# lazytiger/pbrt-rs

Hardware: AMD Instinct MI355X
Metric: Mrays/s (higher is better)
Workload: dtype f32

## Files before the change

### pbrt-rs_amd/csrc/render.hip

```cpp
#include <hip/hip_runtime.h>
#include "abi_guard.h"

#include <algorithm>
#include <chrono>
#include <cstdio>
#include <cstdlib>
#include <cstring>
#include <string>
#include <thread>
#include <vector>

#include "scene.h"
#include "trace.h"
#include "wavefront.h"

using namespace pb;

extern "C" int pbrt_hip_render_device(PbrtHipScene* s, const PbrtCamera* camera, const PbrtRenderParams* params,
                                      float* d_film, PbrtRenderStats* stats) try {
    if (!s || !camera || !params || !d_film) return PBRT_HIP_ERR_INVALID;
    PB_ENTER(s->ctx);
    HIP_TRY(s->ctx, hipSetDevice(s->ctx->device));
    return wavefront_render(s, *camera, *params, d_film, stats);
}
// ... 509 lines not shown
        if (stats) *stats = local;
        return PBRT_HIP_OK;
    }
    const int n_pix = (int)origins.size() * kTile * kTile;
    int64_t valid_pixels = 0;
    for (const int2& o : origins)
        valid_pixels += (int64_t)(std::min(o.x + kTile, rp.x1) - o.x) * (std::min(o.y + kTile, rp.y1) - o.y);
    if (li_mode) valid_pixels = li->n;
    if (export_mode) rp.spp_per_pass = rp.spp;
    int spp_pass = rp.spp_per_pass > 0 ? rp.spp_per_pass : 0;
    if (spp_pass == 0) {
        size_t free_b = 0, total_b = 0;
        HIP_TRY(ctx, hipMemGetInfo(&free_b, &total_b));
        for (const auto& b : ctx->block_cache)
            if (!b.in_use) free_b += b.bytes;
        const int64_t per_path = 400 + (rp.integrator != PBRT_INTEGRATOR_PATH ? 24 + 48ll * std::max(1, rp.max_depth) : 0);
        const int64_t target_paths = std::max<int64_t>(1ll << 20, std::min<int64_t>(1ll << 28, (int64_t)(free_b / 2) / per_path));
        spp_pass = (int)std::max<int64_t>(1, std::min<int64_t>(rp.spp, target_paths / n_pix));
    }
    spp_pass = std::min(spp_pass, rp.spp);
    if (export_mode && spp_pass != rp.spp) return invalid("camera rays: too many samples for one pass");
    const size_t N = (size_t)n_pix * spp_pass;
    if (N * 4 >= (1ull << 32)) return invalid("too many concurrent paths for 32-bit queue entries; lower spp_per_pass");

    DevBuf buf(ctx);
    bool ok = true;
    PathState ps;
    ps.n_paths = N;
    ps.two_level = s->d.bvh.instanced ? 1 : 0;
    ps.ray = buf.alloc<float4>(N * 6, &ok);
    ps.hit = buf.alloc<float4>(N * 6, &ok);
    ps.rng = buf.alloc<uint64_t>(N, &ok);
    ps.L = buf.alloc<float4>(N, &ok);
    ps.beta = buf.alloc<float4>(N, &ok);
    ps.nee_a = buf.alloc<float4>(N, &ok);
    ps.nee_f = buf.alloc<float4>(N, &ok);
    ps.nee_b = buf.alloc<float4>(N, &ok);
    ps.nee_light = buf.alloc<int>(N, &ok);
    ps.pfilm = buf.alloc<float2>(N, &ok);
    Queues q[2];
    for (int k = 0; k < 2; ++k) {
        q[k].trace = buf.alloc<uint32_t>(N * 3, &ok);
        q[k].shade = buf.alloc<uint32_t>(N, &ok);
        q[k].counts64 = buf.alloc<unsigned long long>(2, &ok);
        q[k].keys = nullptr;
        for (int a = 0; a < 3; ++a) {
// ... 462 lines not shown
```

### pbrt-rs_amd/csrc/wf_direct.h

```cpp
#pragma once
#include "wf_path.h"

namespace pb {

struct DirectState {
    int* stage;
    float4* ld_acc;
    float4* frames;
    int light_strategy;
    int mode;
    int ao_samples;
    int ao_cos_sample;
};

#ifndef PB_DIRECT_WAVES
#define PB_DIRECT_WAVES 2
#endif
template <int MODE>
__global__ void __launch_bounds__(256, PB_DIRECT_WAVES) k_shade_direct(ShadeConsts sc, PathState ps, DirectState ds, Queues qin,
                                                        Queues qout, PassParams pp, TileList tiles, uint32_t n_in) {
    uint32_t i = blockIdx.x * blockDim.x + threadIdx.x;
    bool active = i < n_in;
    uint32_t p = active ? qin.shade[i] : 0u;
    bool emit_cont = false, emit_mis = false, emit_shadow = false, mis_bool = false;
    if (active && !(__float_as_int(ps.beta[p].w) & PF_VALID)) active = false;

    if (active) {
        float4 Lq = ps.L[p], bq = ps.beta[p];
        V3 L = V3{Lq.x, Lq.y, Lq.z};
        V3 T = V3{bq.x, bq.y, bq.z};
        int fb = __float_as_int(bq.w);
        int flags = fb & 0xff, depth = fb >> 8;
        int sg = ds.stage[p];
        int stage = sg & 0xffff, sp = sg >> 16;
        float4 accq = ds.ld_acc[p];
        V3 ld_acc = V3{accq.x, accq.y, accq.z};
        size_t rbase = ray_index(ps, p, RS_CONT), hbase = hit_index(ps, p, RS_CONT);
        constexpr int mode = MODE;
        const bool sample_all = mode == PBRT_INTEGRATOR_DIRECT && ds.light_strategy == 0;
        Samp sm = path_sampler(ps, pp, tiles, p);
        const bool tabulated = pp.smp.kind != PBRT_SAMPLER_RANDOM;
        bool fallback = (sm.arr & 0x8000) != 0;
        auto stages_at_vertex = [&]() {
            return (mode == PBRT_INTEGRATOR_AO)        ? ds.ao_samples
                   : (sc.n_lights == 0)                ? 0
                   : (mode == PBRT_INTEGRATOR_WHITTED) ? sc.n_lights
                   : !sample_all                       ? 1
// ... 216 lines not shown
            }
            if (branched) break;
            if (sp == 0) {
                done = true;
                break;
            }
            sp -= 1;
            size_t fi = ((size_t)p * pp.max_depth + sp) * 3;
            float4 f0 = ds.frames[fi], f1 = ds.frames[fi + 1], f2 = ds.frames[fi + 2];
            float4 r0 = ps.ray[rbase];
            ps.ray[rbase] = make_float4(r0.x, r0.y, r0.z, f0.x);
            ps.ray[rbase + 1] = make_float4(f0.y, f0.z, kInf, 0.0f);
            ps.hit[hbase] = make_float4(f1.z, f0.w, f1.x, f1.y);
            if (ps.two_level) ps.hit[hbase + 1] = make_float4(f2.w, 0.0f, 0.0f, 0.0f);
            depth = __float_as_int(f1.w);
            T = V3{f2.x, f2.y, f2.z};
            stage = total + 1;
            surface_ready = false;
            have_vertex = true;
        }
        samp_store(ps, p, sm);
        ps.L[p] = make_float4(L.x, L.y, L.z, 1.0f);
        ps.beta[p] = make_float4(T.x, T.y, T.z, __int_as_float((depth << 8) | flags));
        ds.stage[p] = (stage & 0xffff) | (sp << 16);
        ds.ld_acc[p] = make_float4(ld_acc.x, ld_acc.y, ld_acc.z, 0.0f);
    }

    __shared__ BlockAppend sh;
    block_append(sh, qout, p, emit_cont, emit_mis, emit_shadow, emit_cont || emit_mis || emit_shadow, 0, mis_bool);
}

}
```

### pbrt-rs_amd/csrc/wf_generate_trace.h

```cpp
#pragma once
#include "wf_sampler.h"

namespace pb {

__global__ void k_generate(PathState ps, Queues q, PassParams pp, DevCamera cam, TileList tiles) {
    uint32_t p = blockIdx.x * blockDim.x + threadIdx.x;
    uint32_t n = (uint32_t)pp.n_pix * pp.n_samples;
    if (p >= n) return;
    int s_local, pix;
    path_to_sample_pixel(pp, p, &s_local, &pix);
    int tile = pix >> 8, within = pix & 255;
    int2 org = tiles.origin[tile];
    int x = org.x + (within & 15), y = org.y + (within >> 4);
    bool valid = x >= pp.x0 && x < pp.x1 && y >= pp.y0 && y < pp.y1;
    int flags = 0;
    if (valid) {
        int s = pp.sample0 + s_local;
        Samp sm;
        rng_set_sequence(sm.rng, sample_sequence(pp, x, y, s));
        sm.pix = pix;
        sm.s = s;
        sm.dim1 = sm.dim2 = sm.arr = 0;
        sm.h_offset = pp.smp.kind == PBRT_SAMPLER_HALTON ? halton_pixel_offset(pp.smp, x, y) : 0;
        float u0, u1, l0, l1;
// ... 43 lines not shown
        float xa = __builtin_fabsf(m[0] * o.x) + __builtin_fabsf(m[1] * o.y) + __builtin_fabsf(m[2] * o.z) + __builtin_fabsf(m[3]);
        float ya = __builtin_fabsf(m[4] * o.x) + __builtin_fabsf(m[5] * o.y) + __builtin_fabsf(m[6] * o.z) + __builtin_fabsf(m[7]);
        float za = __builtin_fabsf(m[8] * o.x) + __builtin_fabsf(m[9] * o.y) + __builtin_fabsf(m[10] * o.z) + __builtin_fabsf(m[11]);
        V3 o_err = V3{xa, ya, za} * kGamma3;
        V3 dw = xform_vector(m, d);
        float l2 = len2(dw);
        float tmax = kInf;
        if (l2 > 0.0f) {
            float dt = dot(vabs(dw), o_err) / l2;
            ow = ow + dw * dt;
            tmax -= dt;
        }
        store_ray(ps, p, RS_CONT, ow, dw, tmax);
        samp_store(ps, p, sm);
        ps.pfilm[p] = make_float2(pfx, pfy);
        flags = PF_VALID | PF_ALIVE;
    } else {
        ps.pfilm[p] = make_float2(0.0f, 0.0f);
    }
    ps.L[p] = make_float4(0.0f, 0.0f, 0.0f, 1.0f);
    ps.beta[p] = make_float4(1.0f, 1.0f, 1.0f, __int_as_float(flags));
    if (!valid) store_ray(ps, p, RS_CONT, V3{0.0f, 0.0f, 0.0f}, V3{0.0f, 0.0f, 1.0f}, -1.0f);
    q.trace[p] = p * 4u + RS_CONT;
    q.shade[p] = p;
}

__global__ void k_li_generate(PathState ps, Queues q, const PbrtRay* __restrict__ rays, const uint64_t* __restrict__ keys, uint32_t n,
                              uint32_t n_padded, int skip) {
    uint32_t p = blockIdx.x * blockDim.x + threadIdx.x;
    if (p >= n_padded) return;
    int flags = 0;
    if (p < n) {
        Rng rng;
        rng_set_sequence(rng, keys[p]);
        for (int k = 0; k < skip; ++k) (void)rng_u32(rng);
        ps.rng[p] = rng.state;
        ps.samp[p] = 0;
        const float4* rp = reinterpret_cast<const float4*>(rays + p);
        float4 a = rp[0], b = rp[1];
        store_ray(ps, p, RS_CONT, V3{a.x, a.y, a.z}, V3{a.w, b.x, b.y}, b.z);
        flags = PF_VALID | PF_ALIVE;
    } else {
        store_ray(ps, p, RS_CONT, V3{0.0f, 0.0f, 0.0f}, V3{0.0f, 0.0f, 1.0f}, -1.0f);
    }
    ps.pfilm[p] = make_float2(0.0f, 0.0f);
    ps.L[p] = make_float4(0.0f, 0.0f, 0.0f, 1.0f);
    ps.beta[p] = make_float4(1.0f, 1.0f, 1.0f, __int_as_float(flags));
    q.trace[p] = p * 4u + RS_CONT;
    q.shade[p] = p;
}
__global__ void k_li_output(PathState ps, uint32_t n, float* __restrict__ rgb) {
    uint32_t p = blockIdx.x * blockDim.x + threadIdx.x;
    if (p >= n) return;
    float4 L = ps.L[p];
    rgb[3 * (size_t)p] = L.x;
    rgb[3 * (size_t)p + 1] = L.y;
    rgb[3 * (size_t)p + 2] = L.z;
}
__global__ void k_camera_rays_out(PathState ps, PassParams pp, TileList tiles, PbrtRay* __restrict__ rays, uint64_t* __restrict__ keys,
                                  float* __restrict__ pfilm, int32_t* __restrict__ pixel_sample) {
    uint32_t p = blockIdx.x * blockDim.x + threadIdx.x;
    uint32_t n = (uint32_t)pp.n_pix * pp.n_samples;
    if (p >= n) return;
    int s_local, pix;
    path_to_sample_pixel(pp, p, &s_local, &pix);
    int2 org = tiles.origin[pix >> 8];
    int x = org.x + (pix & 15), y = org.y + ((pix & 255) >> 4);
    bool valid = (__float_as_int(ps.beta[p].w) & PF_VALID) != 0;
    size_t ri = ray_index(ps, p, RS_CONT);
    float4 a = ps.ray[ri], b = ps.ray[ri + 1];
    float4* out = reinterpret_cast<float4*>(rays + p);
    out[0] = a;
// ... 84 lines not shown
```

### pbrt-rs_amd/csrc/wf_lights.h

```cpp
#pragma once
#include "wf_surface.h"

namespace pb {

PB_DEV V3 sphere_through(V3 v) {
    return V3{1.0f * v.x + 0.0f * v.y + 0.0f * v.z, 0.0f * v.x + 1.0f * v.y + 0.0f * v.z, 0.0f * v.x + 0.0f * v.y + 1.0f * v.z};
}
PB_DEV float sphere_area(float radius) { return (360.0f * (kPi / 180.0f)) * radius * (radius - (-radius)); }
PB_DEV void sphere_light_sample(float cx, float cy, float cz, float radius, const Surf& sf, float u0, float u1, V3* p_o,
                                V3* err_o, V3* n_o, float* pdf_o) {
    V3 pc = V3{1.0f * 0.0f + 0.0f * 0.0f + 0.0f * 0.0f + cx, 0.0f * 0.0f + 1.0f * 0.0f + 0.0f * 0.0f + cy,
               0.0f * 0.0f + 0.0f * 0.0f + 1.0f * 0.0f + cz};
    V3 p_origin = offset_ray_origin(sf.p, sf.p_error, sf.n, pc - sf.p);
    if (len2(p_origin - pc) <= radius * radius) {
        float z = 1.0f - 2.0f * u0;
        float rr = __builtin_sqrtf(fmaxr(1.0f - z * z, 0.0f));
        float sp, cp;
        det_sincos(2.0f * kPi * u1, &sp, &cp);
        V3 obj = V3{rr * cp, rr * sp, z} * radius;
        V3 n = normalize(sphere_through(obj));
        obj = obj * (radius / length(obj));
        V3 oe = vabs(obj) * kGamma5;
        const float g3 = kGamma3;
        V3 p = V3{1.0f * obj.x + 0.0f * obj.y + 0.0f * obj.z + cx, 0.0f * obj.x + 1.0f * obj.y + 0.0f * obj.z + cy,
// ... 296 lines not shown
                iu = iu < 0 ? 0 : (iu > 1 ? 1 : iu);
                int iv = (int)(theta * kInvPi * 2.0f);
                iv = iv < 0 ? 0 : (iv > 1 ? 1 : iv);
                lpdf = sc.env_cond_func[iv][iu] / sc.env_marg_int / (2.0f * kPi * kPi * st);
            }
        }
        if (lpdf != 0.0f) {
            float weight = power_heuristic1(spdf, lpdf);
            V3 o2 = offset_ray_origin(sf.p, sf.p_error, sf.n, wi2);
            store_ray(ps, p, RS_MIS, o2, wi2, kInf);
            ps.nee_f[p] = make_float4(f2.x, f2.y, f2.z, weight);
            nee_flags |= PF_NEE_MIS;
            if (sc.mis_bool && lt.type != PBRT_LIGHT_DIFFUSE_AREA) nee_flags |= NEE_MIS_BOOL;
        }
    }
    if (nee_flags) {
        ps.nee_a[p] = make_float4(A.x, A.y, A.z, pick_pdf);
        ps.nee_b[p] = make_float4(beta.x, beta.y, beta.z, spdf);
        ps.nee_light[p] = light_num;
    }
    return nee_flags;
}

PB_DEV V3 estimate_direct_resolve(const ShadeConsts& sc, const PathState& ps, uint32_t p, int flags, float* pick_pdf,
                                  V3* beta_at_vertex) {
    float4 na = ps.nee_a[p], nf = ps.nee_f[p], nb = ps.nee_b[p];
    int light_id = ps.nee_light[p];
    V3 ld = V3{0.0f, 0.0f, 0.0f};
    if (flags & PF_NEE_SHADOW) {
        bool occluded = ps.hit[hit_index(ps, p, RS_SHADOW)].x != 0.0f;
        if (!occluded) ld = ld + V3{na.x, na.y, na.z};
    }
    if (flags & PF_NEE_MIS) {
        int hslot = __float_as_int(ps.hit[hit_index(ps, p, RS_MIS)].x);
        DevLight lt = sc.lights[light_id];
        V3 li = V3{0.0f, 0.0f, 0.0f};
        if (hslot >= 0) {
            int hl = lt.type == PBRT_LIGHT_DIFFUSE_AREA ? (__float_as_int(sc.bvh.tris[3 * (size_t)hslot + 2].w) & kPrimLightMask) - 1 : -2;
            if (hl == light_id) {
                float4 r0 = ps.ray[ray_index(ps, p, RS_MIS)], r1 = ps.ray[ray_index(ps, p, RS_MIS) + 1];
                V3 wi = V3{r0.w, r1.x, r1.y};
                float4 hb = ps.hit[hit_index(ps, p, RS_MIS)];
                V3 n = tri_interaction_normal(sc.bvh, hslot, hb.y, hb.z, hb.w);
                if (lt.two_sided || dot(n, -wi) > 0.0f) li = V3{lt.L[0], lt.L[1], lt.L[2]};
            }
        } else if (lt.type == PBRT_LIGHT_INFINITE) {
            li = V3{lt.L[0], lt.L[1], lt.L[2]};
        }
        if (!is_black(li)) {
            V3 f = V3{nf.x, nf.y, nf.z};
            ld = ld + mulv(li, f) * nf.w / nb.w;
        }
    }
    *pick_pdf = na.w;
    *beta_at_vertex = V3{nb.x, nb.y, nb.z};
    return ld;
}

PB_DEV V3 sample_specular_local(const DevMaterial& mat, V3 kd, V3 kt, V3 wol, float ur, int which, V3* wil, float* pdf,
                                bool* transmission) {
    *pdf = 0.0f;
    *transmission = false;
    V3 zero = V3{0.0f, 0.0f, 0.0f};
    if (mat.type == PBRT_MAT_MIRROR) {
        if (which == 2 || is_black(kd)) return zero;
        *wil = V3{-wol.x, -wol.y, wol.z};
        *pdf = 1.0f;
        return mulv(kd, V3{1.0f, 1.0f, 1.0f}) / __builtin_fabsf(wil->z);
    }
    if (mat.type != PBRT_MAT_GLASS) return zero;
    if (which == 0) {
        float F = fr_dielectric(wol.z, 1.0f, mat.eta);
        if (ur < F) {
            *wil = V3{-wol.x, -wol.y, wol.z};
            *pdf = F;
            return kd * F / __builtin_fabsf(wil->z);
        }
        bool entering = wol.z > 0.0f;
        float eta_i = entering ? 1.0f : mat.eta, eta_t = entering ? mat.eta : 1.0f;
// ... 28 lines not shown
```

### pbrt-rs_amd/csrc/wf_path.h

```cpp
#pragma once
#include "wf_lights.h"

namespace pb {

PB_DEV uint32_t shade_key(const ShadeConsts& sc, const PathState& ps, uint32_t p, int max_depth) {
    int fb = __float_as_int(ps.beta[p].w);
    uint32_t key = 0;
    if ((fb & PF_ALIVE) && (fb >> 8) < max_depth) {
        const size_t hb = hit_index(ps, p, RS_CONT);
        int slot = __float_as_int(ps.hit[hb].x), inst = hit_instance(ps, hb);
        if (slot >= 0) {
            int mat = __float_as_int(sc.bvh.tris[3 * (size_t)slot + 2].z);
            if (sc.bvh.instanced && inst >= 0) {
                int over = __float_as_int(sc.bvh.instances[7 * (size_t)inst + 6].x);
                if (over >= 0) mat = over;
            }
            key = 1u + (uint32_t)sc.materials[mat].type;
        }
    }
    return key;
}
__global__ void k_shade_sort_keys(ShadeConsts sc, PathState ps, const uint32_t* __restrict__ shade_queue, uint32_t n, int max_depth,
                                  uint32_t* __restrict__ keys) {
    uint32_t i = blockIdx.x * blockDim.x + threadIdx.x;
    if (i >= n) return;
    keys[i] = shade_key(sc, ps, shade_queue[i], max_depth);
}

constexpr int kShadeKeys = 6;
struct ShadeBins {
    uint32_t count[4][kShadeKeys];
    uint32_t path[256];
};

#ifndef PB_SHADE_WAVES
#define PB_SHADE_WAVES 3
#endif
template <bool BIN>
__global__ void __launch_bounds__(256, PB_SHADE_WAVES) k_shade(ShadeConsts sc, PathState ps, Queues qin, Queues qout, PassParams pp,
                                                 TileList tiles, uint32_t n_in) {
    uint32_t i = blockIdx.x * blockDim.x + threadIdx.x;
    bool active = i < n_in;
    uint32_t p = active ? qin.shade[i] : 0u;
    if (BIN) {
        __shared__ ShadeBins bins;
        const int lane = threadIdx.x & 63, wave = threadIdx.x >> 6;
        const uint32_t key = active ? shade_key(sc, ps, p, pp.max_depth) : (uint32_t)(kShadeKeys - 1);
        uint32_t rank = 0;
#pragma unroll
        for (int k = 0; k < kShadeKeys; ++k) {
            const unsigned long long m = __ballot(key == (uint32_t)k);
            if (key == (uint32_t)k) rank = lane_prefix(m);
            if (lane == 0) bins.count[wave][k] = (uint32_t)__popcll(m);
        }
        __syncthreads();
        uint32_t before = 0;
        for (int k = 0; k < kShadeKeys; ++k)
            for (int w = 0; w < 4; ++w)
                before += ((uint32_t)k < key || ((uint32_t)k == key && w < wave)) ? bins.count[w][k] : 0u;
        bins.path[before + rank] = p;
        uint32_t n_active = 0;
        for (int k = 0; k < kShadeKeys - 1; ++k)
            for (int w = 0; w < 4; ++w) n_active += bins.count[w][k];
        __syncthreads();
        p = bins.path[threadIdx.x];
        active = threadIdx.x < n_active;
    }
    bool emit_cont = false, emit_mis = false, emit_shadow = false, mis_bool = false;

    uint32_t cell = 0;
    if (active) {
        float4 Lq = ps.L[p], bq = ps.beta[p];
        V3 L = V3{Lq.x, Lq.y, Lq.z};
        float eta_scale = Lq.w;
        V3 beta = V3{bq.x, bq.y, bq.z};
        int fb = __float_as_int(bq.w);
        int flags = fb & 0xff, bounces = fb >> 8;
        size_t rbase = ray_index(ps, p, RS_CONT), hbase = hit_index(ps, p, RS_CONT);

        if (flags & (PF_NEE_SHADOW | PF_NEE_MIS)) {
            float pick_pdf;
            V3 beta_v;
            V3 ld = estimate_direct_resolve(sc, ps, p, flags, &pick_pdf, &beta_v);
            ld = ld / pick_pdf;
            L = L + mulv(beta_v, ld);
            flags &= ~(PF_NEE_SHADOW | PF_NEE_MIS);
        }

        if (flags & PF_ALIVE) {
            flags &= ~PF_ALIVE;
            float4 r0 = ps.ray[rbase], r1 = ps.ray[rbase + 1];
            V3 rd = V3{r0.w, r1.x, r1.y};
            float4 h0 = ps.hit[hbase];
            int hslot = __float_as_int(h0.x);
            bool found = hslot >= 0;
            Surf sf;
            if (found) {
                sf = surface_from_hit(sc.bvh, hslot, hit_instance(ps, hbase), h0.y, h0.z, h0.w, rd);
                if (qout.keys) cell = ray_sort_cell(sf.p.x, sf.p.y, sf.p.z, qout.key_lo, qout.key_inv);
            }
            if (bounces == 0 || (flags & PF_SPECULAR_BOUNCE)) {
                if (found) {
                    L = L + mulv(beta, surface_le(sc, sf, -rd));
                } else {
                    for (int k = 0; k < sc.n_infinite; ++k) {
                        DevLight lt = sc.lights[sc.infinite_ids[k]];
                        L = L + mulv(beta, V3{lt.L[0], lt.L[1], lt.L[2]});
                    }
                }
            }
            if (found && bounces < pp.max_depth) {
                DevMaterial mat = sc.materials[sf.material];
                Samp sm = path_sampler(ps, pp, tiles, p);
                if (mat.type == PBRT_MAT_NONE) {
                    V3 o = offset_ray_origin(sf.p, sf.p_error, sf.n, rd);
                    store_ray(ps, p, RS_CONT, o, rd, kInf);
                    flags |= PF_ALIVE;
                    emit_cont = true;
                } else {
                    Frame fr = make_frame(sf);
                    V3 kd = V3{mat.kd[0], mat.kd[1], mat.kd[2]};
                    V3 kt = V3{mat.kt[0], mat.kt[1], mat.kt[2]};
                    V3 wo = -rd;
                    bool has_lobe;
                    if (mat.type == PBRT_MAT_GLASS) has_lobe = !(is_black(kd) && is_black(kt));
                    else has_lobe = !is_black(kd);
                    bool nonspecular = (mat.type == PBRT_MAT_MATTE) && has_lobe;

                    if (nonspecular && sc.n_lights > 0) {
                        float u_pick = samp_1d(pp, sm);
                        DevDistribution1D distrib = light_distribution_lookup(sc, sf.p);
                        int light_num = find_interval_cdf(distrib.cdf, distrib.n + 1, u_pick);
                        float pick_pdf = distrib.func_int > 0.0f ? distrib.func[light_num] / (distrib.func_int * (float)distrib.n)
                                                                 : 0.0f;
                        if (pick_pdf != 0.0f) {
                            float ul0, ul1, us0, us1;
// ... 42 lines not shown
                        V3 rr_beta = beta * eta_scale;
                        if (max_comp(rr_beta) < pp.rr_threshold && bounces > 3) {
                            float qq = fmaxr(0.05f, 1.0f - max_comp(rr_beta));
                            if (samp_1d(pp, sm) < qq) alive = false;
                            else beta = beta / (1.0f - qq);
                        }
                        if (alive) {
                            store_ray(ps, p, RS_CONT, o, wi, kInf);
                            flags |= PF_ALIVE;
                            emit_cont = true;
                            bounces += 1;
                        }
                    }
                }
                samp_store(ps, p, sm);
            }
        }
        ps.L[p] = make_float4(L.x, L.y, L.z, eta_scale);
        ps.beta[p] = make_float4(beta.x, beta.y, beta.z, __int_as_float((bounces << 8) | flags));
    }

    __shared__ BlockAppend sh;
    const bool again = emit_cont || emit_mis || emit_shadow;
    block_append(sh, qout, p, emit_cont, emit_mis, emit_shadow, again, cell, mis_bool);
}

}
```

### pbrt-rs_amd/csrc/wf_state.h

```cpp
#pragma once
#include <hip/hip_runtime.h>

#include "scene.h"
#include "trace.h"
#include "trace_persistent.h"
#include "trace_wide.h"
#include "trace_stackless.h"

namespace pb {

constexpr int kTile = 16;
enum PathFlags : int {
    PF_SPECULAR_BOUNCE = 1,
    PF_ALIVE = 2,
    PF_NEE_SHADOW = 4,
    PF_NEE_MIS = 8,
    PF_VALID = 16,
};
enum RaySlot : int { RS_CONT = 0, RS_MIS = 1, RS_SHADOW = 2 };
constexpr uint32_t RS_MIS_BOOL = 3;
constexpr int NEE_MIS_BOOL = 0x100;

struct PathState {
    float4* ray;
    float4* hit;
    size_t n_paths;
    uint64_t* rng;
    float4* L;
    float4* beta;
    float4* nee_a;
    float4* nee_f;
    float4* nee_b;
    int* nee_light;
    float2* pfilm;
    int* samp;
    int two_level;
};
PB_DEV int hit_instance(const PathState& ps, size_t hit_base) { return ps.two_level ? __float_as_int(ps.hit[hit_base + 1].x) : -1; }

#ifndef PB_RAY_PATH_MAJOR
#define PB_RAY_PATH_MAJOR 0
#endif
#ifndef PB_HIT_PATH_MAJOR
#define PB_HIT_PATH_MAJOR 0
// ... 74 lines not shown
                     (uint32_t)fminf(fmaxf(fz * kCells, 0.0f), kCells - 1.0f)};
    uint32_t code = 0;
    for (int b = 0; b < PB_SORT_AXIS_BITS; ++b)
        for (int k = 0; k < 3; ++k) code |= ((q[k] >> b) & 1u) << (3 * b + k);
    return code;
}

PB_DEV int64_t pixel_number(const PassParams& pp, int x, int y) {
    return (int64_t)(y - pp.sb_y0) * pp.sb_w + (x - pp.sb_x0);
}
PB_DEV uint64_t sample_sequence(const PassParams& pp, int x, int y, int s) {
    return pp.seed ^ (uint64_t)(pixel_number(pp, x, y) * (int64_t)pp.spp + s);
}

struct BlockAppend {
    uint32_t wave_rays[16];
    uint32_t wave_shadow[16];
    uint32_t wave_paths[16];
    uint32_t base_rays, base_paths;
};
PB_DEV uint32_t lane_prefix(unsigned long long mask) {
    return __builtin_amdgcn_mbcnt_hi((uint32_t)(mask >> 32), __builtin_amdgcn_mbcnt_lo((uint32_t)mask, 0));
}
PB_DEV void block_append(BlockAppend& sh, const Queues& q, uint32_t p, bool cont, bool mis, bool shadow, bool again,
                         uint32_t cell = 0, bool mis_bool = false) {
    const int lane = threadIdx.x & 63, wave = threadIdx.x >> 6, n_waves = (blockDim.x + 63) >> 6;
    unsigned long long mc = __ballot(cont), mm = __ballot(mis), ms = __ballot(shadow), ma = __ballot(again);
    uint32_t wc = (uint32_t)__popcll(mc), wm = (uint32_t)__popcll(mm), ws = (uint32_t)__popcll(ms);
    if (lane == 0) {
        sh.wave_rays[wave] = wc + wm + ws;
        sh.wave_shadow[wave] = ws;
        sh.wave_paths[wave] = (uint32_t)__popcll(ma);
    }
    __syncthreads();
    if (threadIdx.x == 0) {
        uint32_t tr = 0, tsd = 0, tp = 0;
        for (int w = 0; w < n_waves; ++w) {
            uint32_t r = sh.wave_rays[w], pth = sh.wave_paths[w];
            sh.wave_rays[w] = tr;
            sh.wave_paths[w] = tp;
            tr += r;
            tsd += sh.wave_shadow[w];
            tp += pth;
        }
        unsigned long long old = 0;
        if (tr) old = atomicAdd(&q.counts64[0], (unsigned long long)tr | ((unsigned long long)tsd << 32));
        sh.base_rays = (uint32_t)old;
        sh.base_paths = tp ? (uint32_t)atomicAdd(&q.counts64[1], (unsigned long long)tp) : 0u;
    }
    __syncthreads();
    uint32_t rbase = sh.base_rays + sh.wave_rays[wave];
    uint32_t ic = rbase + lane_prefix(mc), im = rbase + wc + lane_prefix(mm), is = rbase + wc + wm + lane_prefix(ms);
    if (cont) q.trace[ic] = p * 4u + RS_CONT;
    if (mis) q.trace[im] = p * 4u + (mis_bool ? RS_MIS_BOOL : (uint32_t)RS_MIS);
    if (shadow) q.trace[is] = p * 4u + RS_SHADOW;
    if (q.keys) {
        if (cont) q.keys[ic] = cell;
        if (mis) q.keys[im] = mis_bool ? (cell | (1u << (kSortKeyBits - 1))) : cell;
        if (shadow) q.keys[is] = cell | (1u << (kSortKeyBits - 1));
    }
    if (again) q.shade[sh.base_paths + sh.wave_paths[wave] + lane_prefix(ma)] = p;
}

PB_DEV void store_ray(const PathState& ps, uint32_t p, int slot, V3 o, V3 d, float tmax) {
    size_t i = ray_index(ps, p, slot);
    ps.ray[i] = make_float4(o.x, o.y, o.z, d.x);
    ps.ray[i + 1] = make_float4(d.y, d.z, tmax, 0.0f);
}

struct DevCamera {
    float c2w[16], r2c[16];
    float lens_radius, focal_distance, shutter_open, shutter_close;
    int kind;
};
PB_DEV V3 xform_point(const float* m, V3 p) {
    float xp = m[0] * p.x + m[1] * p.y + m[2] * p.z + m[3];
    float yp = m[4] * p.x + m[5] * p.y + m[6] * p.z + m[7];
    float zp = m[8] * p.x + m[9] * p.y + m[10] * p.z + m[11];
    float wp = m[12] * p.x + m[13] * p.y + m[14] * p.z + m[15];
    if (wp == 1.0f) return V3{xp, yp, zp};
    return V3{xp, yp, zp} / wp;
}
PB_DEV V3 xform_vector(const float* m, V3 v) {
    return V3{m[0] * v.x + m[1] * v.y + m[2] * v.z, m[4] * v.x + m[5] * v.y + m[6] * v.z,
// ... 10 lines not shown
```

### pbrt-rs_amd/csrc/wf_surface.h

```cpp
#pragma once
#include "wf_generate_trace.h"

namespace pb {

struct Surf {
    V3 p, p_error, n, dpdu, wo;
    V3 ns, sdpdu;
    int material, light;
};

PB_DEV void tri_vertices(const DevBVH& bvh, int slot, V3* p0, V3* p1, V3* p2, int* prim, int* mat, int* light) {
    float4 a = bvh.tris[3 * (size_t)slot], b = bvh.tris[3 * (size_t)slot + 1], c = bvh.tris[3 * (size_t)slot + 2];
    *p0 = V3{a.x, a.y, a.z};
    *p1 = V3{a.w, b.x, b.y};
    *p2 = V3{b.z, b.w, c.x};
    *prim = __float_as_int(c.y);
    *mat = __float_as_int(c.z);
    *light = (__float_as_int(c.w) & kPrimLightMask) - 1;
}

PB_DEV void tri_shading_geometry(const DevBVH& bvh, int slot, V3 p0, V3 p1, V3 p2, float b0, float b1, float b2, V3* n_out,
                                 V3* ns_out, V3* dpdu_out, V3* sdpdu_out) {
    float uv0x = 0.0f, uv0y = 0.0f, uv1x = 1.0f, uv1y = 0.0f, uv2x = 1.0f, uv2y = 1.0f;
    float4 s0 = make_float4(0, 0, 0, 0), s1 = s0, s2 = s0, s3 = s0, s4 = s0;
    if (bvh.tri_shading) {
        const float4* sh = bvh.tri_shading + 6 * (size_t)slot;
        s0 = sh[0];
        s1 = sh[1];
        s2 = sh[2];
        s3 = sh[3];
        s4 = sh[4];
        if (bvh.has_uvs) {
            float4 s5 = sh[5];
            uv0x = s4.z;
            uv0y = s4.w;
            uv1x = s5.x;
            uv1y = s5.y;
            uv2x = s5.z;
            uv2y = s5.w;
        }
    }
// ... 22 lines not shown
        }
        V3 ss = normalize(dpdu);
        if (bvh.has_tangents) {
            V3 t0 = V3{s2.y, s2.z, s2.w}, t1 = V3{s3.x, s3.y, s3.z}, t2 = V3{s3.w, s4.x, s4.y};
            V3 si = t0 * b0 + t1 * b1 + t2 * b2;
            if (len2(si) > 0.0f) ss = normalize(si);
        }
        V3 ts = cross(ss, nsi);
        if (len2(ts) > 0.0f) {
            ts = normalize(ts);
            ss = cross(ts, nsi);
        } else {
            coordinate_system(nsi, &ss, &ts);
        }
        ns = normalize(cross(ss, ts));
        if (dot(n, ns) < 0.0f) n = -n;
        sdpdu = ss;
    }
    *n_out = n;
    *ns_out = ns;
    *dpdu_out = dpdu;
    *sdpdu_out = sdpdu;
}
PB_DEV Surf make_surface(const DevBVH& bvh, int slot, float b0, float b1, float b2, V3 ray_d) {
    V3 p0, p1, p2;
    int prim;
    Surf s;
    tri_vertices(bvh, slot, &p0, &p1, &p2, &prim, &s.material, &s.light);
    tri_shading_geometry(bvh, slot, p0, p1, p2, b0, b1, b2, &s.n, &s.ns, &s.dpdu, &s.sdpdu);
    float xs = __builtin_fabsf(b0 * p0.x) + __builtin_fabsf(b1 * p1.x) + __builtin_fabsf(b2 * p2.x);
    float ys = __builtin_fabsf(b0 * p0.y) + __builtin_fabsf(b1 * p1.y) + __builtin_fabsf(b2 * p2.y);
    float zs = __builtin_fabsf(b0 * p0.z) + __builtin_fabsf(b1 * p1.z) + __builtin_fabsf(b2 * p2.z);
    s.p_error = V3{xs, ys, zs} * kGamma7;
    s.p = p0 * b0 + p1 * b1 + p2 * b2;
    s.wo = -ray_d;
    return s;
}
PB_DEV void instance_to_world(const DevBVH& bvh, int inst_slot, Surf* s) {
    const float4* m = bvh.instances + 7 * (size_t)inst_slot;
    float4 o0 = m[0], o1 = m[1], o2 = m[2];
    float4 w0 = m[3], w1 = m[4], w2 = m[5];
    V3 p = s->p, pe = s->p_error;
    float xp = w0.x * p.x + w0.y * p.y + w0.z * p.z + w0.w;
    float yp = w1.x * p.x + w1.y * p.y + w1.z * p.z + w1.w;
    float zp = w2.x * p.x + w2.y * p.y + w2.z * p.z + w2.w;
    const float g3 = kGamma3;
    V3 err;
    err.x = (g3 + 1.0f) * (__builtin_fabsf(w0.x * pe.x) + __builtin_fabsf(w0.y * pe.y) + __builtin_fabsf(w0.z * pe.z)) +
            g3 * (__builtin_fabsf(w0.x * p.x) + __builtin_fabsf(w0.y * p.y) + __builtin_fabsf(w0.z * p.z) + __builtin_fabsf(w0.w));
    err.y = (g3 + 1.0f) * (__builtin_fabsf(w1.x * pe.x) + __builtin_fabsf(w1.y * pe.y) + __builtin_fabsf(w1.z * pe.z)) +
            g3 * (__builtin_fabsf(w1.x * p.x) + __builtin_fabsf(w1.y * p.y) + __builtin_fabsf(w1.z * p.z) + __builtin_fabsf(w1.w));
// ... 39 lines not shown
    V3 n = normalize(cross(dpdu, dpdv));
    V3 pe = vabs(ph) * kGamma5;
    const float g3 = kGamma3;
    float x = ph.x, y = ph.y, z = ph.z;
    s.p = V3{1.0f * x + 0.0f * y + 0.0f * z + cx, 0.0f * x + 1.0f * y + 0.0f * z + cy, 0.0f * x + 0.0f * y + 1.0f * z + cz};
    s.p_error.x = (g3 + 1.0f) * (__builtin_fabsf(1.0f * pe.x) + __builtin_fabsf(0.0f * pe.y) + __builtin_fabsf(0.0f * pe.z)) +
                  g3 * (__builtin_fabsf(1.0f * x) + __builtin_fabsf(0.0f * y) + __builtin_fabsf(0.0f * z) + __builtin_fabsf(cx));
    s.p_error.y = (g3 + 1.0f) * (__builtin_fabsf(0.0f * pe.x) + __builtin_fabsf(1.0f * pe.y) + __builtin_fabsf(0.0f * pe.z)) +
                  g3 * (__builtin_fabsf(0.0f * x) + __builtin_fabsf(1.0f * y) + __builtin_fabsf(0.0f * z) + __builtin_fabsf(cy));
    s.p_error.z = (g3 + 1.0f) * (__builtin_fabsf(0.0f * pe.x) + __builtin_fabsf(0.0f * pe.y) + __builtin_fabsf(1.0f * pe.z)) +
                  g3 * (__builtin_fabsf(0.0f * x) + __builtin_fabsf(0.0f * y) + __builtin_fabsf(1.0f * z) + __builtin_fabsf(cz));
    auto through = [](V3 v) {
        return V3{1.0f * v.x + 0.0f * v.y + 0.0f * v.z, 0.0f * v.x + 1.0f * v.y + 0.0f * v.z, 0.0f * v.x + 0.0f * v.y + 1.0f * v.z};
    };
    s.n = normalize(through(n));
    V3 d_obj = through(rd);
    s.wo = normalize(through(-d_obj));
    s.dpdu = through(dpdu);
    V3 sn = normalize(through(n));
    s.ns = dot(sn, s.n) < 0.0f ? -sn : sn;
    s.sdpdu = through(dpdu);
    return s;
}
PB_DEV Surf surface_from_hit(const DevBVH& bvh, int slot, int inst_slot, float b0, float b1, float b2, V3 rd) {
    if (bvh.has_spheres && (__float_as_int(bvh.tris[3 * (size_t)slot + 2].w) & kPrimSphere))
        return make_surface_sphere(bvh, slot, V3{b0, b1, b2}, rd);
    if (bvh.instanced && inst_slot >= 0) {
        const float4* m = bvh.instances + 7 * (size_t)inst_slot;
        float4 r0 = m[0], r1 = m[1], r2 = m[2];
        V3 d_obj = V3{r0.x * rd.x + r0.y * rd.y + r0.z * rd.z, r1.x * rd.x + r1.y * rd.y + r1.z * rd.z,
                      r2.x * rd.x + r2.y * rd.y + r2.z * rd.z};
        Surf s = make_surface(bvh, slot, b0, b1, b2, d_obj);
        instance_to_world(bvh, inst_slot, &s);
        return s;
    }
    return make_surface(bvh, slot, b0, b1, b2, rd);
}
PB_DEV V3 tri_interaction_normal(const DevBVH& bvh, int slot, float b0, float b1, float b2) {
    if (bvh.has_spheres && (__float_as_int(bvh.tris[3 * (size_t)slot + 2].w) & kPrimSphere))
        return make_surface_sphere(bvh, slot, V3{b0, b1, b2}, V3{0.0f, 0.0f, 1.0f}).n;
    V3 p0, p1, p2;
    int a, b, c;
    tri_vertices(bvh, slot, &p0, &p1, &p2, &a, &b, &c);
    if (!(bvh.tri_shading && (bvh.has_normals || bvh.has_tangents))) return normalize(cross(p0 - p2, p1 - p2));
    V3 n, ns, dpdu, sdpdu;
    tri_shading_geometry(bvh, slot, p0, p1, p2, b0, b1, b2, &n, &ns, &dpdu, &sdpdu);
    return n;
}

struct Frame {
    V3 ss, ts, ns, ng;
};
PB_DEV V3 to_local(const Frame& f, V3 v) { return V3{dot(v, f.ss), dot(v, f.ts), dot(v, f.ns)}; }
PB_DEV V3 to_world(const Frame& f, V3 v) {
    return V3{f.ss.x * v.x + f.ts.x * v.y + f.ns.x * v.z, f.ss.y * v.x + f.ts.y * v.y + f.ns.y * v.z,
              f.ss.z * v.x + f.ts.z * v.y + f.ns.z * v.z};
}

PB_DEV void matte_f_pdf(const Frame& fr, V3 kd, V3 wo_w, V3 wi_w, V3* f, float* pdf) {
// ... 88 lines not shown
};

PB_DEV DevDistribution1D light_distribution_lookup(const ShadeConsts& sc, V3 p) {
    if (!sc.spatial) return sc.distrib;
    const float* mn = sc.bvh.root_min;
    const float* mx = sc.bvh.root_max;
    float o[3] = {p.x - mn[0], p.y - mn[1], p.z - mn[2]};
    int pi[3];
    for (int i = 0; i < 3; ++i) {
        if (mx[i] > mn[i]) o[i] /= mx[i] - mn[i];
        int v = (int)(o[i] * (float)sc.n_voxel[i]);
        pi[i] = v < 0 ? 0 : (v > sc.n_voxel[i] - 1 ? sc.n_voxel[i] - 1 : v);
    }
    size_t voxel = ((size_t)pi[2] * sc.n_voxel[1] + pi[1]) * sc.n_voxel[0] + pi[0];
    const float* t = sc.spatial + voxel * (size_t)(2 * sc.n_lights + 2);
    DevDistribution1D d;
    d.func = t;
    d.cdf = t + sc.n_lights;
    d.func_int = t[2 * sc.n_lights + 1];
    d.n = sc.n_lights;
    return d;
}

PB_DEV Samp path_sampler(const PathState& ps, const PassParams& pp, const TileList& tiles, uint32_t p) {
    Samp sm;
    if (pp.stream_keys) {
        sm.rng.inc = (pp.stream_keys[p] << 1) | 1;
        sm.rng.state = ps.rng[p];
        sm.pix = 0;
        sm.s = 0;
        sm.dim1 = sm.dim2 = sm.arr = 0;
        sm.h_offset = 0;
        return sm;
    }
    int s_local, pix;
    path_to_sample_pixel(pp, p, &s_local, &pix);
    int2 org = tiles.origin[pix >> 8];
    int x = org.x + (pix & 15), y = org.y + ((pix & 255) >> 4);
    sm.rng.inc = (sample_sequence(pp, x, y, pp.sample0 + s_local) << 1) | 1;
    sm.rng.state = ps.rng[p];
    sm.pix = pix;
    sm.s = pp.sample0 + s_local;
    int c = ps.samp[p];
    sm.dim1 = c & 0x3ff;
    sm.dim2 = (c >> 10) & 0x3f;
    sm.arr = (c >> 16) & 0xffff;
    sm.h_offset = pp.smp.kind == PBRT_SAMPLER_HALTON ? halton_pixel_offset(pp.smp, x, y) : 0;
    return sm;
}

PB_DEV Frame make_frame(const Surf& sf) {
    Frame fr;
    fr.ns = sf.ns;
    fr.ng = sf.n;
    fr.ss = normalize(sf.sdpdu);
    fr.ts = cross(fr.ns, fr.ss);
    return fr;
}

PB_DEV V3 surface_le(const ShadeConsts& sc, const Surf& sf, V3 w) {
    if (sf.light >= 0) {
        DevLight lt = sc.lights[sf.light];
        if (lt.two_sided || dot(sf.n, w) > 0.0f) return V3{lt.L[0], lt.L[1], lt.L[2]};
    }
    return V3{0.0f, 0.0f, 0.0f};
}

}
```

Baseline: 2834.

## Pack path flags into shade queue entries and hoist shade-kernel loads

Shade queue entries now carry the path's NEE/alive/specular flags in their top bits, so the path shade kernel knows up front which state to fetch. It then issues all dependent global loads (NEE records, shadow/MIS hits, ray, hit, triangle record, light, sampler words) together at kernel entry, using clamped index 0 for inactive branches, instead of scattering them behind branches. This aims to increase memory-level parallelism and hide load latency. In exchange it adds redundant loads of slot 0, higher register pressure, and caps concurrent paths at 2^28.

```diff
diff --git a/pbrt-rs_amd/csrc/render.hip b/pbrt-rs_amd/csrc/render.hip
--- a/pbrt-rs_amd/csrc/render.hip
+++ b/pbrt-rs_amd/csrc/render.hip
@@ -555,6 +555,8 @@
     if (export_mode && spp_pass != rp.spp) return invalid("camera rays: too many samples for one pass");
     const size_t N = (size_t)n_pix * spp_pass;
     if (N * 4 >= (1ull << 32)) return invalid("too many concurrent paths for 32-bit queue entries; lower spp_per_pass");
+    if (N > ((size_t)1 << pb::kShadeFlagShift))
+        return invalid("too many concurrent paths for the shade queue (2^28 at most: the path flags ride above the path number); lower spp_per_pass");
 
     DevBuf buf(ctx);
     bool ok = true;
diff --git a/pbrt-rs_amd/csrc/wf_direct.h b/pbrt-rs_amd/csrc/wf_direct.h
--- a/pbrt-rs_amd/csrc/wf_direct.h
+++ b/pbrt-rs_amd/csrc/wf_direct.h
@@ -21,8 +21,9 @@
                                                         Queues qout, PassParams pp, TileList tiles, uint32_t n_in) {
     uint32_t i = blockIdx.x * blockDim.x + threadIdx.x;
     bool active = i < n_in;
-    uint32_t p = active ? qin.shade[i] : 0u;
+    uint32_t p = active ? shade_path(qin.shade[i]) : 0u;
     bool emit_cont = false, emit_mis = false, emit_shadow = false, mis_bool = false;
+    int flags_out = 0;
     if (active && !(__float_as_int(ps.beta[p].w) & PF_VALID)) active = false;
 
     if (active) {
@@ -285,12 +286,13 @@
         samp_store(ps, p, sm);
         ps.L[p] = make_float4(L.x, L.y, L.z, 1.0f);
         ps.beta[p] = make_float4(T.x, T.y, T.z, __int_as_float((depth << 8) | flags));
+        flags_out = flags;
         ds.stage[p] = (stage & 0xffff) | (sp << 16);
         ds.ld_acc[p] = make_float4(ld_acc.x, ld_acc.y, ld_acc.z, 0.0f);
     }
 
     __shared__ BlockAppend sh;
-    block_append(sh, qout, p, emit_cont, emit_mis, emit_shadow, emit_cont || emit_mis || emit_shadow, 0, mis_bool);
+    block_append(sh, qout, p, flags_out, emit_cont, emit_mis, emit_shadow, emit_cont || emit_mis || emit_shadow, 0, mis_bool);
 }
 
 }
diff --git a/pbrt-rs_amd/csrc/wf_generate_trace.h b/pbrt-rs_amd/csrc/wf_generate_trace.h
--- a/pbrt-rs_amd/csrc/wf_generate_trace.h
+++ b/pbrt-rs_amd/csrc/wf_generate_trace.h
@@ -89,7 +89,7 @@
     ps.beta[p] = make_float4(1.0f, 1.0f, 1.0f, __int_as_float(flags));
     if (!valid) store_ray(ps, p, RS_CONT, V3{0.0f, 0.0f, 0.0f}, V3{0.0f, 0.0f, 1.0f}, -1.0f);
     q.trace[p] = p * 4u + RS_CONT;
-    q.shade[p] = p;
+    q.shade[p] = shade_entry(p, flags);
 }
 
 __global__ void k_li_generate(PathState ps, Queues q, const PbrtRay* __restrict__ rays, const uint64_t* __restrict__ keys, uint32_t n,
@@ -114,7 +114,7 @@
     ps.L[p] = make_float4(0.0f, 0.0f, 0.0f, 1.0f);
     ps.beta[p] = make_float4(1.0f, 1.0f, 1.0f, __int_as_float(flags));
     q.trace[p] = p * 4u + RS_CONT;
-    q.shade[p] = p;
+    q.shade[p] = shade_entry(p, flags);
 }
 __global__ void k_li_output(PathState ps, uint32_t n, float* __restrict__ rgb) {
     uint32_t p = blockIdx.x * blockDim.x + threadIdx.x;
diff --git a/pbrt-rs_amd/csrc/wf_lights.h b/pbrt-rs_amd/csrc/wf_lights.h
--- a/pbrt-rs_amd/csrc/wf_lights.h
+++ b/pbrt-rs_amd/csrc/wf_lights.h
@@ -342,25 +342,42 @@
     return nee_flags;
 }
 
-PB_DEV V3 estimate_direct_resolve(const ShadeConsts& sc, const PathState& ps, uint32_t p, int flags, float* pick_pdf,
-                                  V3* beta_at_vertex) {
-    float4 na = ps.nee_a[p], nf = ps.nee_f[p], nb = ps.nee_b[p];
-    int light_id = ps.nee_light[p];
+struct NeePending {
+    float4 a, f, b;
+    int light;
+    float shadow;
+    float4 mis_hit;
+};
+PB_DEV NeePending nee_pending_load(const PathState& ps, uint32_t p, int flags) {
+    const uint32_t pn = (flags & (PF_NEE_SHADOW | PF_NEE_MIS)) ? p : 0u, psh = (flags & PF_NEE_SHADOW) ? p : 0u,
+                   pm = (flags & PF_NEE_MIS) ? p : 0u;
+    NeePending ne;
+    ne.a = ps.nee_a[pn];
+    ne.f = ps.nee_f[pn];
+    ne.b = ps.nee_b[pn];
+    ne.light = ps.nee_light[pn];
+    ne.shadow = ps.hit[hit_index(ps, psh, RS_SHADOW)].x;
+    ne.mis_hit = ps.hit[hit_index(ps, pm, RS_MIS)];
+    return ne;
+}
+PB_DEV V3 estimate_direct_resolve(const ShadeConsts& sc, const PathState& ps, uint32_t p, int flags, const NeePending& ne,
+                                  const DevLight& lt, float* pick_pdf, V3* beta_at_vertex) {
+    const float4 na = ne.a, nf = ne.f, nb = ne.b;
+    const int light_id = ne.light;
     V3 ld = V3{0.0f, 0.0f, 0.0f};
     if (flags & PF_NEE_SHADOW) {
-        bool occluded = ps.hit[hit_index(ps, p, RS_SHADOW)].x != 0.0f;
+        bool occluded = ne.shadow != 0.0f;
         if (!occluded) ld = ld + V3{na.x, na.y, na.z};
     }
     if (flags & PF_NEE_MIS) {
-        int hslot = __float_as_int(ps.hit[hit_index(ps, p, RS_MIS)].x);
-        DevLight lt = sc.lights[light_id];
+        int hslot = __float_as_int(ne.mis_hit.x);
         V3 li = V3{0.0f, 0.0f, 0.0f};
         if (hslot >= 0) {
             int hl = lt.type == PBRT_LIGHT_DIFFUSE_AREA ? (__float_as_int(sc.bvh.tris[3 * (size_t)hslot + 2].w) & kPrimLightMask) - 1 : -2;
             if (hl == light_id) {
                 float4 r0 = ps.ray[ray_index(ps, p, RS_MIS)], r1 = ps.ray[ray_index(ps, p, RS_MIS) + 1];
                 V3 wi = V3{r0.w, r1.x, r1.y};
-                float4 hb = ps.hit[hit_index(ps, p, RS_MIS)];
+                float4 hb = ne.mis_hit;
                 V3 n = tri_interaction_normal(sc.bvh, hslot, hb.y, hb.z, hb.w);
                 if (lt.two_sided || dot(n, -wi) > 0.0f) li = V3{lt.L[0], lt.L[1], lt.L[2]};
             }
@@ -375,6 +392,13 @@
     *pick_pdf = na.w;
     *beta_at_vertex = V3{nb.x, nb.y, nb.z};
     return ld;
+}
+PB_DEV V3 estimate_direct_resolve(const ShadeConsts& sc, const PathState& ps, uint32_t p, int flags, float* pick_pdf,
+                                  V3* beta_at_vertex) {
+    const NeePending ne = nee_pending_load(ps, p, flags);
+    DevLight lt{};
+    if (flags & PF_NEE_MIS) lt = sc.lights[ne.light];
+    return estimate_direct_resolve(sc, ps, p, flags, ne, lt, pick_pdf, beta_at_vertex);
 }
 
 PB_DEV V3 sample_specular_local(const DevMaterial& mat, V3 kd, V3 kt, V3 wol, float ur, int which, V3* wil, float* pdf,
diff --git a/pbrt-rs_amd/csrc/wf_path.h b/pbrt-rs_amd/csrc/wf_path.h
--- a/pbrt-rs_amd/csrc/wf_path.h
+++ b/pbrt-rs_amd/csrc/wf_path.h
@@ -1,9 +1,13 @@
 #pragma once
 #include "wf_lights.h"
+#ifdef PB_CHECK_SHADE_FLAGS
+#include <cassert>
+#endif
 
 namespace pb {
 
-PB_DEV uint32_t shade_key(const ShadeConsts& sc, const PathState& ps, uint32_t p, int max_depth) {
+PB_DEV uint32_t shade_key(const ShadeConsts& sc, const PathState& ps, uint32_t entry, int max_depth) {
+    const uint32_t p = shade_path(entry);
     int fb = __float_as_int(ps.beta[p].w);
     uint32_t key = 0;
     if ((fb & PF_ALIVE) && (fb >> 8) < max_depth) {
@@ -41,11 +45,11 @@
                                                  TileList tiles, uint32_t n_in) {
     uint32_t i = blockIdx.x * blockDim.x + threadIdx.x;
     bool active = i < n_in;
-    uint32_t p = active ? qin.shade[i] : 0u;
+    uint32_t entry = active ? qin.shade[i] : 0u;
     if (BIN) {
         __shared__ ShadeBins bins;
         const int lane = threadIdx.x & 63, wave = threadIdx.x >> 6;
-        const uint32_t key = active ? shade_key(sc, ps, p, pp.max_depth) : (uint32_t)(kShadeKeys - 1);
+        const uint32_t key = active ? shade_key(sc, ps, entry, pp.max_depth) : (uint32_t)(kShadeKeys - 1);
         uint32_t rank = 0;
 #pragma unroll
         for (int k = 0; k < kShadeKeys; ++k) {
@@ -58,30 +62,56 @@
         for (int k = 0; k < kShadeKeys; ++k)
             for (int w = 0; w < 4; ++w)
                 before += ((uint32_t)k < key || ((uint32_t)k == key && w < wave)) ? bins.count[w][k] : 0u;
-        bins.path[before + rank] = p;
+        bins.path[before + rank] = entry;
         uint32_t n_active = 0;
         for (int k = 0; k < kShadeKeys - 1; ++k)
             for (int w = 0; w < 4; ++w) n_active += bins.count[w][k];
         __syncthreads();
-        p = bins.path[threadIdx.x];
+        entry = bins.path[threadIdx.x];
         active = threadIdx.x < n_active;
     }
+    const uint32_t p = shade_path(entry);
+    const int qflags = shade_flags(entry);
     bool emit_cont = false, emit_mis = false, emit_shadow = false, mis_bool = false;
 
     uint32_t cell = 0;
+    int flags = 0;
     if (active) {
-        float4 Lq = ps.L[p], bq = ps.beta[p];
+        const float4 Lq = ps.L[p], bq = ps.beta[p];
+        const NeePending ne = nee_pending_load(ps, p, qflags);
+        const uint32_t pc = (qflags & PF_ALIVE) ? p : 0u;
+        const size_t rbase = ray_index(ps, pc, RS_CONT), hbase = hit_index(ps, pc, RS_CONT);
+        const float4 r0 = ps.ray[rbase], r1 = ps.ray[rbase + 1];
+        const V3 rd = V3{r0.w, r1.x, r1.y};
+        const float4 h0 = ps.hit[hbase];
+        const int hinst = hit_instance(ps, hbase);
+        const SampWords sw = path_sampler_load(ps, pp, tiles, pc);
         V3 L = V3{Lq.x, Lq.y, Lq.z};
         float eta_scale = Lq.w;
         V3 beta = V3{bq.x, bq.y, bq.z};
         int fb = __float_as_int(bq.w);
-        int flags = fb & 0xff, bounces = fb >> 8;
-        size_t rbase = ray_index(ps, p, RS_CONT), hbase = hit_index(ps, p, RS_CONT);
+        flags = fb & 0xff;
+        int bounces = fb >> 8;
+#ifdef PB_CHECK_SHADE_FLAGS
+        assert((flags & kShadeQueueFlags) == qflags);
+#endif
+
+        const int hslot = __float_as_int(h0.x);
+        const bool found = hslot >= 0;
+        const bool hit = (qflags & PF_ALIVE) && found;
+        DevBVH tb = sc.bvh;
+        if (tb.n_slots == 0) tb.tris = ps.ray;
+        float4 trec[3];
+        tri_record(tb, hit ? hslot : 0, trec);
+        const DevLight* lights = sc.n_lights > 0 ? sc.lights : reinterpret_cast<const DevLight*>(ps.ray);
+        const DevLight lt = lights[(qflags & PF_NEE_MIS) ? ne.light : 0];
+        const Surf sf = surface_from_hit(tb, hit ? hslot : 0, trec, hit ? hinst : -1, h0.y, h0.z, h0.w, rd);
+        if ((flags & PF_ALIVE) && found && qout.keys) cell = ray_sort_cell(sf.p.x, sf.p.y, sf.p.z, qout.key_lo, qout.key_inv);
 
         if (flags & (PF_NEE_SHADOW | PF_NEE_MIS)) {
             float pick_pdf;
             V3 beta_v;
-            V3 ld = estimate_direct_resolve(sc, ps, p, flags, &pick_pdf, &beta_v);
+            V3 ld = estimate_direct_resolve(sc, ps, p, flags, ne, lt, &pick_pdf, &beta_v);
             ld = ld / pick_pdf;
             L = L + mulv(beta_v, ld);
             flags &= ~(PF_NEE_SHADOW | PF_NEE_MIS);
@@ -89,16 +119,6 @@
 
         if (flags & PF_ALIVE) {
             flags &= ~PF_ALIVE;
-            float4 r0 = ps.ray[rbase], r1 = ps.ray[rbase + 1];
-            V3 rd = V3{r0.w, r1.x, r1.y};
-            float4 h0 = ps.hit[hbase];
-            int hslot = __float_as_int(h0.x);
-            bool found = hslot >= 0;
-            Surf sf;
-            if (found) {
-                sf = surface_from_hit(sc.bvh, hslot, hit_instance(ps, hbase), h0.y, h0.z, h0.w, rd);
-                if (qout.keys) cell = ray_sort_cell(sf.p.x, sf.p.y, sf.p.z, qout.key_lo, qout.key_inv);
-            }
             if (bounces == 0 || (flags & PF_SPECULAR_BOUNCE)) {
                 if (found) {
                     L = L + mulv(beta, surface_le(sc, sf, -rd));
@@ -111,7 +131,7 @@
             }
             if (found && bounces < pp.max_depth) {
                 DevMaterial mat = sc.materials[sf.material];
-                Samp sm = path_sampler(ps, pp, tiles, p);
+                Samp sm = path_sampler(pp, sw);
                 if (mat.type == PBRT_MAT_NONE) {
                     V3 o = offset_ray_origin(sf.p, sf.p_error, sf.n, rd);
                     store_ray(ps, p, RS_CONT, o, rd, kInf);
@@ -200,7 +220,7 @@
 
     __shared__ BlockAppend sh;
     const bool again = emit_cont || emit_mis || emit_shadow;
-    block_append(sh, qout, p, emit_cont, emit_mis, emit_shadow, again, cell, mis_bool);
-}
-
-}
+    block_append(sh, qout, p, flags, emit_cont, emit_mis, emit_shadow, again, cell, mis_bool);
+}
+
+}
diff --git a/pbrt-rs_amd/csrc/wf_state.h b/pbrt-rs_amd/csrc/wf_state.h
--- a/pbrt-rs_amd/csrc/wf_state.h
+++ b/pbrt-rs_amd/csrc/wf_state.h
@@ -20,6 +20,13 @@
 enum RaySlot : int { RS_CONT = 0, RS_MIS = 1, RS_SHADOW = 2 };
 constexpr uint32_t RS_MIS_BOOL = 3;
 constexpr int NEE_MIS_BOOL = 0x100;
+constexpr int kShadeFlagShift = 28;
+constexpr uint32_t kShadePathMask = (1u << kShadeFlagShift) - 1u;
+constexpr int kShadeQueueFlags = PF_SPECULAR_BOUNCE | PF_ALIVE | PF_NEE_SHADOW | PF_NEE_MIS;
+static_assert((kShadeQueueFlags >> (32 - kShadeFlagShift)) == 0, "the queued path flags must fit above the path number");
+PB_DEV uint32_t shade_entry(uint32_t p, int flags) { return p | ((uint32_t)(flags & kShadeQueueFlags) << kShadeFlagShift); }
+PB_DEV uint32_t shade_path(uint32_t entry) { return entry & kShadePathMask; }
+PB_DEV int shade_flags(uint32_t entry) { return (int)(entry >> kShadeFlagShift); }
 
 struct PathState {
     float4* ray;
@@ -140,7 +147,7 @@
 PB_DEV uint32_t lane_prefix(unsigned long long mask) {
     return __builtin_amdgcn_mbcnt_hi((uint32_t)(mask >> 32), __builtin_amdgcn_mbcnt_lo((uint32_t)mask, 0));
 }
-PB_DEV void block_append(BlockAppend& sh, const Queues& q, uint32_t p, bool cont, bool mis, bool shadow, bool again,
+PB_DEV void block_append(BlockAppend& sh, const Queues& q, uint32_t p, int flags, bool cont, bool mis, bool shadow, bool again,
                          uint32_t cell = 0, bool mis_bool = false) {
     const int lane = threadIdx.x & 63, wave = threadIdx.x >> 6, n_waves = (blockDim.x + 63) >> 6;
     unsigned long long mc = __ballot(cont), mm = __ballot(mis), ms = __ballot(shadow), ma = __ballot(again);
@@ -177,7 +184,7 @@
         if (mis) q.keys[im] = mis_bool ? (cell | (1u << (kSortKeyBits - 1))) : cell;
         if (shadow) q.keys[is] = cell | (1u << (kSortKeyBits - 1));
     }
-    if (again) q.shade[sh.base_paths + sh.wave_paths[wave] + lane_prefix(ma)] = p;
+    if (again) q.shade[sh.base_paths + sh.wave_paths[wave] + lane_prefix(ma)] = shade_entry(p, flags);
 }
 
 PB_DEV void store_ray(const PathState& ps, uint32_t p, int slot, V3 o, V3 d, float tmax) {
diff --git a/pbrt-rs_amd/csrc/wf_surface.h b/pbrt-rs_amd/csrc/wf_surface.h
--- a/pbrt-rs_amd/csrc/wf_surface.h
+++ b/pbrt-rs_amd/csrc/wf_surface.h
@@ -9,14 +9,25 @@
     int material, light;
 };
 
-PB_DEV void tri_vertices(const DevBVH& bvh, int slot, V3* p0, V3* p1, V3* p2, int* prim, int* mat, int* light) {
-    float4 a = bvh.tris[3 * (size_t)slot], b = bvh.tris[3 * (size_t)slot + 1], c = bvh.tris[3 * (size_t)slot + 2];
+PB_DEV void tri_vertices(const float4 (&rec)[3], V3* p0, V3* p1, V3* p2, int* prim, int* mat, int* light) {
+    const float4 a = rec[0], b = rec[1], c = rec[2];
     *p0 = V3{a.x, a.y, a.z};
     *p1 = V3{a.w, b.x, b.y};
     *p2 = V3{b.z, b.w, c.x};
     *prim = __float_as_int(c.y);
     *mat = __float_as_int(c.z);
     *light = (__float_as_int(c.w) & kPrimLightMask) - 1;
+}
+PB_DEV void tri_record(const DevBVH& bvh, int slot, float4 (&rec)[3]) {
+    const float4* t = bvh.tris + 3 * (size_t)slot;
+    rec[0] = t[0];
+    rec[1] = t[1];
+    rec[2] = t[2];
+}
+PB_DEV void tri_vertices(const DevBVH& bvh, int slot, V3* p0, V3* p1, V3* p2, int* prim, int* mat, int* light) {
+    float4 rec[3];
+    tri_record(bvh, slot, rec);
+    tri_vertices(rec, p0, p1, p2, prim, mat, light);
 }
 
 PB_DEV void tri_shading_geometry(const DevBVH& bvh, int slot, V3 p0, V3 p1, V3 p2, float b0, float b1, float b2, V3* n_out,
@@ -85,11 +96,11 @@
     *dpdu_out = dpdu;
     *sdpdu_out = sdpdu;
 }
-PB_DEV Surf make_surface(const DevBVH& bvh, int slot, float b0, float b1, float b2, V3 ray_d) {
+PB_DEV Surf make_surface(const DevBVH& bvh, int slot, const float4 (&rec)[3], float b0, float b1, float b2, V3 ray_d) {
     V3 p0, p1, p2;
     int prim;
     Surf s;
-    tri_vertices(bvh, slot, &p0, &p1, &p2, &prim, &s.material, &s.light);
+    tri_vertices(rec, &p0, &p1, &p2, &prim, &s.material, &s.light);
     tri_shading_geometry(bvh, slot, p0, p1, p2, b0, b1, b2, &s.n, &s.ns, &s.dpdu, &s.sdpdu);
     float xs = __builtin_fabsf(b0 * p0.x) + __builtin_fabsf(b1 * p1.x) + __builtin_fabsf(b2 * p2.x);
     float ys = __builtin_fabsf(b0 * p0.y) + __builtin_fabsf(b1 * p1.y) + __builtin_fabsf(b2 * p2.y);
@@ -175,19 +186,24 @@
     s.sdpdu = through(dpdu);
     return s;
 }
-PB_DEV Surf surface_from_hit(const DevBVH& bvh, int slot, int inst_slot, float b0, float b1, float b2, V3 rd) {
-    if (bvh.has_spheres && (__float_as_int(bvh.tris[3 * (size_t)slot + 2].w) & kPrimSphere))
+PB_DEV Surf surface_from_hit(const DevBVH& bvh, int slot, const float4 (&rec)[3], int inst_slot, float b0, float b1, float b2, V3 rd) {
+    if (bvh.has_spheres && (__float_as_int(rec[2].w) & kPrimSphere))
         return make_surface_sphere(bvh, slot, V3{b0, b1, b2}, rd);
     if (bvh.instanced && inst_slot >= 0) {
         const float4* m = bvh.instances + 7 * (size_t)inst_slot;
         float4 r0 = m[0], r1 = m[1], r2 = m[2];
         V3 d_obj = V3{r0.x * rd.x + r0.y * rd.y + r0.z * rd.z, r1.x * rd.x + r1.y * rd.y + r1.z * rd.z,
                       r2.x * rd.x + r2.y * rd.y + r2.z * rd.z};
-        Surf s = make_surface(bvh, slot, b0, b1, b2, d_obj);
+        Surf s = make_surface(bvh, slot, rec, b0, b1, b2, d_obj);
         instance_to_world(bvh, inst_slot, &s);
         return s;
     }
-    return make_surface(bvh, slot, b0, b1, b2, rd);
+    return make_surface(bvh, slot, rec, b0, b1, b2, rd);
+}
+PB_DEV Surf surface_from_hit(const DevBVH& bvh, int slot, int inst_slot, float b0, float b1, float b2, V3 rd) {
+    float4 rec[3];
+    tri_record(bvh, slot, rec);
+    return surface_from_hit(bvh, slot, rec, inst_slot, b0, b1, b2, rd);
 }
 PB_DEV V3 tri_interaction_normal(const DevBVH& bvh, int slot, float b0, float b1, float b2) {
     if (bvh.has_spheres && (__float_as_int(bvh.tris[3 * (size_t)slot + 2].w) & kPrimSphere))
@@ -322,31 +338,49 @@
     return d;
 }
 
-PB_DEV Samp path_sampler(const PathState& ps, const PassParams& pp, const TileList& tiles, uint32_t p) {
+struct SampWords {
+    uint64_t state;
+    uint64_t key;
+    int counters;
+    int s_local, pix;
+    int2 org;
+};
+PB_DEV SampWords path_sampler_load(const PathState& ps, const PassParams& pp, const TileList& tiles, uint32_t p) {
+    SampWords w;
+    path_to_sample_pixel(pp, p, &w.s_local, &w.pix);
+    w.state = ps.rng[p];
+    w.counters = ps.samp[p];
+    w.org = tiles.origin[w.pix >> 8];
+    w.key = pp.stream_keys ? pp.stream_keys[p] : 0;
+    return w;
+}
+PB_DEV Samp path_sampler(const PassParams& pp, const SampWords& w) {
     Samp sm;
     if (pp.stream_keys) {
-        sm.rng.inc = (pp.stream_keys[p] << 1) | 1;
-        sm.rng.state = ps.rng[p];
+        sm.rng.inc = (w.key << 1) | 1;
+        sm.rng.state = w.state;
         sm.pix = 0;
         sm.s = 0;
         sm.dim1 = sm.dim2 = sm.arr = 0;
         sm.h_offset = 0;
         return sm;
     }
-    int s_local, pix;
-    path_to_sample_pixel(pp, p, &s_local, &pix);
-    int2 org = tiles.origin[pix >> 8];
+    const int s_local = w.s_local, pix = w.pix;
+    int2 org = w.org;
     int x = org.x + (pix & 15), y = org.y + ((pix & 255) >> 4);
     sm.rng.inc = (sample_sequence(pp, x, y, pp.sample0 + s_local) << 1) | 1;
-    sm.rng.state = ps.rng[p];
+    sm.rng.state = w.state;
     sm.pix = pix;
     sm.s = pp.sample0 + s_local;
-    int c = ps.samp[p];
+    int c = w.counters;
     sm.dim1 = c & 0x3ff;
     sm.dim2 = (c >> 10) & 0x3f;
     sm.arr = (c >> 16) & 0xffff;
     sm.h_offset = pp.smp.kind == PBRT_SAMPLER_HALTON ? halton_pixel_offset(pp.smp, x, y) : 0;
     return sm;
+}
+PB_DEV Samp path_sampler(const PathState& ps, const PassParams& pp, const TileList& tiles, uint32_t p) {
+    return path_sampler(pp, path_sampler_load(ps, pp, tiles, p));
 }
 
 PB_DEV Frame make_frame(const Surf& sf) {
```

Result: no change. 2831, median of 2 (-0.1%).
